# ErikBrorsson/MVDet

Hardware: AMD Instinct MI355X
Metric: multi-view frames/sec (project+fuse) (higher is better)
Workload: dtype f32 (3xbf16-split products hi*hi+hi*lo+lo*hi on the bf16 MFMA, fp32 accumulate)

## Files before the change

### mvdet_amd/csrc/conv_bf16x3.hip

```cpp
#include "common.h"

#include <type_traits>

namespace mvbev {
namespace b3 {

typedef float floatx16 __attribute__((ext_vector_type(16)));
typedef float floatx4 __attribute__((ext_vector_type(4)));
typedef __bf16 bf16x8 __attribute__((ext_vector_type(8)));
typedef unsigned int u32x4 __attribute__((ext_vector_type(4)));

constexpr int SB = MVBEV_CONV_KC;
constexpr int KC = 2 * SB;
constexpr int NKB = 9;
constexpr int BN = MVBEV_CONV_BN;
constexpr int TW = 32;
constexpr int WPART = NKB * KC * BN;
constexpr int WBYTES = 2 * WPART * 2;
constexpr int W16 = WBYTES / 16;

__global__ void pack_kernel(const float* __restrict__ w, __bf16* __restrict__ out, int Cout,
                            int Cin_w, const int32_t* __restrict__ chan_map, int K, int K_pad) {
  const int n_cot = Cout / BN;
  const int64_t total = (int64_t)(K_pad / KC) * n_cot * 2 * WPART;
// ... 1208 lines not shown
  const int col = x0 + c, r3 = 4 * ty + q;
  if (col >= W) return;
  const int base = 12 * ty + (a.dil == 1 ? 3 * q : ring_base_row<2>(q));
  int64_t roff[5];
  bool rok[5];
#pragma unroll
  for (int m = 0; m < 5; ++m) {
    const int row = a.out_row0 + base + a.dil * (m - 1), by = row - a.in_row0;
    rok[m] = row >= 0 && row < a.H && by >= 0 && by < a.in_rows;
    roff[m] = 2 * ((int64_t)by * W + col);
  }
  u32x4 raw[4][5][2];
#pragma unroll
  for (int i = 0; i < 4; ++i) {
    const int kb = kb0 + kq + 2 * i;
    const bool kok = kb < nb && g * a.group + kb * SB < a.K;
    const u32x4* src = a.x + ((int64_t)b * a.batch_stride + (int64_t)g * a.group_stride +
                              (int64_t)(kok ? kb : 0) * SB * plane) / 4;
#pragma unroll
    for (int m = 0; m < 5; ++m)
#pragma unroll
      for (int p = 0; p < 2; ++p) raw[i][m][p] = (kok && rok[m]) ? src[roff[m] + p] : u32x4{0u, 0u, 0u, 0u};
  }
#pragma unroll
  for (int i = 0; i < 4; ++i) {
    const int kb = kb0 + kq + 2 * i, k0 = g * a.group + kb * SB;
    if (kb >= nb || k0 >= a.K) continue;
    float d[5][8];
#pragma unroll
    for (int m = 0; m < 5; ++m) {
      float h[8], l[8];
      bf16x8_to_f32(raw[i][m][0], h);
      bf16x8_to_f32(raw[i][m][1], l);
#pragma unroll
      for (int j = 0; j < 8; ++j) d[m][j] = h[j] + l[j];
    }
    u32x4* dst = a.t + 2 * (((int64_t)b * K8 + k0 / SB) * R5 * W + (int64_t)5 * r3 * W) + col;
#pragma unroll
    for (int xi = 0; xi < 5; ++xi) {
      unsigned hp[4], lp[4];
#pragma unroll
      for (int e4 = 0; e4 < 4; ++e4) {
        unsigned short hs[2], ls[2];
#pragma unroll
        for (int e = 0; e < 2; ++e) {
          const int j = 2 * e4 + e;
          const float d0 = d[0][j], d1 = d[1][j], d2 = d[2][j], d3 = d[3][j], d4 = d[4][j];
          const float v = xi == 0 ? 2.f * d0 - d1 - 2.f * d2 + d3
                        : xi == 1 ? -2.f * d1 - d2 + d3
                        : xi == 2 ? 2.f * d1 - 3.f * d2 + d3
                        : xi == 3 ? d3 - d1
                                  : 2.f * d1 - d2 - 2.f * d3 + d4;
          const __bf16 hv = (__bf16)v, lv = (__bf16)(v - (float)hv);
          hs[e] = __builtin_bit_cast(unsigned short, hv);
          ls[e] = __builtin_bit_cast(unsigned short, lv);
        }
        hp[e4] = (unsigned)hs[0] | ((unsigned)hs[1] << 16);
        lp[e4] = (unsigned)ls[0] | ((unsigned)ls[1] << 16);
      }
      dst[2 * (int64_t)xi * W] = u32x4{hp[0], hp[1], hp[2], hp[3]};
      dst[2 * (int64_t)xi * W + W] = u32x4{lp[0], lp[1], lp[2], lp[3]};
    }
  }
}

#ifndef MVBEV_WINO_STAMPS
#define MVBEV_WINO_STAMPS 0
#endif
#if MVBEV_WINO_STAMPS
__device__ long long g_wino_stamps[4 * 65536];
#endif
__device__ __attribute__((always_inline)) inline void init_to_m(floatx16 (&acc)[2][wino::NXI]) {
#pragma unroll
  for (int ct = 0; ct < 2; ++ct)
#pragma unroll
    for (int r = 0; r < 16; ++r) {
      const float i0 = acc[ct][0][r], i1 = acc[ct][1][r], i2 = acc[ct][2][r];
      acc[ct][0][r] = i0 - i2;
      acc[ct][1][r] = 0.5f * (i1 + i2);
      acc[ct][2][r] = 0.5f * (i2 - i1);
    }
}

template <bool RELU, int DIL, bool P3>
__global__ __launch_bounds__(RNT, 1) void conv_wino_kernel(const Args a) {
  using namespace wino;
  using G = Geo<DIL>;
#if MVBEV_WINO_STAMPS
  const long long stamp0 = wall_clock64();
#endif
  constexpr int XW = G::XW, TROW = G::TROW, NXT = G::NXT;
  __shared__ __attribute__((aligned(16))) u32x4 lds[LDS];
  const int W = a.W;
  const int tid = threadIdx.x, lane = tid & 63;
  const int wave = __builtin_amdgcn_readfirstlane(tid >> 6);
  const int l32 = lane & 31, kl = lane >> 5;

  int tile = xcd_remap(blockIdx.x, a.nwg);
  if (a.gmask) {
    const int Gq = a.mgroup;
    const int x = blockIdx.x & 7, j = blockIdx.x >> 3;
    const int q = j / a.n_cot;
    const int slot = Gq * (8 * (q / Gq) + x) + q % Gq;
    if (slot >= a.npix) return;
    tile = (a.tile_order ? a.tile_order[slot] : slot) * a.n_cot + j % a.n_cot;
  }
  const int cot = tile % a.n_cot, rest = tile / a.n_cot;
  const int t_main = a.tiles_y * a.tiles_x;
  const int pp = rest % t_main, b = rest / t_main;
  const int ty = pp / a.tiles_x;
  const int x0 = (pp - ty * a.tiles_x) * TW;
  const int y0 = a.out_row0 + ty * RT;
  if (a.cmask && !((a.cmask[pp] >> (cot / a.cot_pg)) & 1u)) return;
  const uint32_t gm = a.gmask ? a.gmask[pp] : 0u;
  const int nch = a.gmask ? __builtin_popcount(gm) * a.cpg : a.nchunks;
  const int K8 = a.K / SB;
  const int64_t tplane2 = 2LL * (XH * a.tiles_y) * W;
  const uint32_t tplane_b = (uint32_t)(tplane2 * 16);
  constexpr uint32_t kOOB = 0x80000000u;
  uint32_t wvo[NWI], tvo[NXTMAX];
#pragma unroll
  for (int j = 0; j < NWI; ++j) {
    const int e = (j * NIW + wave) * 64 + lane;
    wvo[j] = (uint32_t)(((e / RHALF) * (NTAP * 2 * BN) + e % RHALF) * 16);
    asm volatile("" : "+v"(wvo[j]));
  }
#pragma unroll
  for (int j = 0; j < NXT; ++j) {
    const int e = (j * NIW + wave) * 64 + lane;
    const int sub = e / (TROW / 2), part = (e / (TROW / 4)) & 1, rt = (e % (TROW / 4)) / XW, c = e % XW;
    const int gx = x0 - DIL + c;
    const bool z = e >= TROW || gx < 0 || gx >= W;
    tvo[j] = z ? kOOB : (uint32_t)sub * tplane_b + (uint32_t)((2 * (XH * ty + NXI * rt) * W + part * W + gx) * 16);
    asm volatile("" : "+v"(tvo[j]));
  }
  const int cpg = a.gmask ? a.cpg : max(nch, 1);
  uint32_t rem = a.gmask ? gm : 1u;
  int gbase = a.gmask ? __builtin_ctz(gm | 0x80000000u) * cpg : 0, ci = 0, wi = 0;
  auto step = [&]() __attribute__((always_inline)) {
    if (wi + 1 < nch) {
      ++wi;
      if (++ci == cpg) {
        ci = 0;
        rem &= rem - 1;
        gbase = __builtin_ctz(rem | 0x80000000u) * cpg;
      }
    }
    return gbase + ci;
  };
  const char* wcot = reinterpret_cast<const char*>(a.wp + (int64_t)cot * wino::W16);
  const char* tb0 = reinterpret_cast<const char*>(static_cast<const u32x4*>(a.x) + (int64_t)b * K8 * tplane2);
  struct ChunkBase {
    const char* w;
    const char* t;
    bool kv1;
  };
  auto base_of = [&](int ph) __attribute__((always_inline)) {
    return ChunkBase{wcot + (int64_t)ph * a.n_cot * wino::W16 * 16, tb0 + (int64_t)(2 * ph) * tplane2 * 16,
                     2 * ph + 1 < K8};
  };
  auto issue_unit = [&](const ChunkBase& cb, int xi, int slot) __attribute__((always_inline)) {
    if (wave >= NIW) return;
    u32x4* dst = lds + slot * SLOT + wave * 64;
    const __amdgpu_buffer_rsrc_t rw =
        __builtin_amdgcn_make_buffer_rsrc(const_cast<char*>(cb.w + xi * 3 * 2 * BN * 16), (short)0, 0x7fffffff, 0x00020000);
#pragma unroll
    for (int j = 0; j < NWI; ++j)
      __builtin_amdgcn_raw_ptr_buffer_load_lds(rw, (__attribute__((address_space(3))) void*)(dst + j * NIT), 16,
                                               wvo[j], 0, 0, 0);
    const int32_t rows_b = xi * W * 32;
    const __amdgpu_buffer_rsrc_t rt = __builtin_amdgcn_make_buffer_rsrc(
        const_cast<char*>(cb.t + rows_b), (short)0, cb.kv1 ? 0x7fffffff : (int)(tplane_b - rows_b), 0x00020000);
#pragma unroll
    for (int j = 0; j < NXT; ++j)
      if ((j * NIW + wave) * 64 < TROW)
        __builtin_amdgcn_raw_ptr_buffer_load_lds(rt, (__attribute__((address_space(3))) void*)(dst + RUNIT + j * NIT),
                                                 16, tvo[j], 0, 0, 0);
  };
  ChunkBase cur = base_of(gbase + ci);
  ChunkBase nx = base_of(step());
  auto advance = [&]() __attribute__((always_inline)) {
    cur = nx;
    nx = base_of(step());
  };

  const int rg = wave & 3;
  const int cw = 64 * (wave >> 2);
  floatx16 acc[2][NXI];
#pragma unroll
  for (int i = 0; i < 2; ++i)
#pragma unroll
    for (int j = 0; j < NXI; ++j) acc[i][j] = floatx16{0};
  if constexpr (!P3) {
    if (a.init) load_init<3>(a, y0 + ring_base_row<DIL>(rg), DIL, x0 + l32, cot * BN + cw, acc);
  }
  bf16x8 fb[3][2];
  bf16x8 fa[2][2][2];
  auto fetch_b = [&](int kw, int slot) __attribute__((always_inline)) {
    const u32x4* X = lds + slot * SLOT + RUNIT + kl * (TROW / 2) + rg * XW + l32 + DIL * kw;
#pragma unroll
    for (int p = 0; p < 2; ++p) fb[kw][p] = __builtin_bit_cast(bf16x8, X[p * (TROW / 4)]);
  };
  auto fetch_a = [&](int st, int slot, int kw) __attribute__((always_inline)) {
    const u32x4* Wl = lds + slot * SLOT + kw * 2 * BN + kl * BN + cw + l32;
#pragma unroll
    for (int ct = 0; ct < 2; ++ct)
#pragma unroll
      for (int p = 0; p < 2; ++p) fa[st][ct][p] = __builtin_bit_cast(bf16x8, Wl[p * RHALF + 32 * ct]);
  };
  auto sched6 = [&](auto nreads) __attribute__((always_inline)) {
    constexpr int n = decltype(nreads)::value;
#pragma unroll
    for (int i = 0; i < 6; ++i) {
      __builtin_amdgcn_sched_group_barrier(0x008, 1, 0);
      if (i < n) __builtin_amdgcn_sched_group_barrier(0x100, (n + 5) / 6, 0);
    }
  };

  constexpr int NXT_LO = TROW / NIT;
  constexpr int WHI = (TROW % NIT + 63) / 64;
  static_assert(NXT_LO + (WHI > 0) == NXT, "T pieces");
  constexpr int NPU_HI = NWI + NXT;
  constexpr int NPU_LO = NWI + NXT_LO;
  const bool whi = wave < WHI;
#ifndef MVBEV_WINO_PB2
#define MVBEV_WINO_PB2 1
#endif
  constexpr bool PB = DIL == 2 && MVBEV_WINO_PB2;
  if (nch > 0) {
    const int U = NXI * nch;
    issue_unit(cur, 0, 0);
    issue_unit(cur, 1, 1);
    issue_unit(cur, 2, 2);
    issue_unit(cur, 3, 3);
    if (PB) {
      if (whi) asm volatile("s_waitcnt vmcnt(%0)" ::"n"(2 * NPU_HI) : "memory");
      else asm volatile("s_waitcnt vmcnt(%0)" ::"n"(2 * NPU_LO) : "memory");
    } else {
      if (whi) asm volatile("s_waitcnt vmcnt(%0)" ::"n"(3 * NPU_HI) : "memory");
      else asm volatile("s_waitcnt vmcnt(%0)" ::"n"(3 * NPU_LO) : "memory");
    }
    __builtin_amdgcn_s_barrier();
    asm volatile("" ::: "memory");
    if constexpr (!P3) init_to_m(acc);
    fetch_b(0, 0);
    fetch_b(1, 0);
    fetch_a(0, 0, 0);
#define WINO_MFMAS(AS, KW, XI)                                                                       \
  _Pragma("unroll") for (int ct = 0; ct < 2; ++ct) {                                                 \
    acc[ct][XI] = __builtin_amdgcn_mfma_f32_32x32x16_bf16(fa[AS][ct][1], fb[KW][0], acc[ct][XI], 0, 0, 0); \
    acc[ct][XI] = __builtin_amdgcn_mfma_f32_32x32x16_bf16(fa[AS][ct][0], fb[KW][1], acc[ct][XI], 0, 0, 0); \
    acc[ct][XI] = __builtin_amdgcn_mfma_f32_32x32x16_bf16(fa[AS][ct][0], fb[KW][0], acc[ct][XI], 0, 0, 0); \
  }
#define WINO_UNIT(R)                                                                                 \
  do {                                                                                               \
    constexpr int XI = (R) % 5, P = (R) & 1;                                                          \
    if (u0 + (R) >= U) break;                                                                        \
    constexpr int slot = (R) & 3, nslot = ((R) + 1) & 3;                         \
    fetch_a(P ^ 1, slot, 1);                                                                         \
    fetch_b(2, slot);                                                                                \
    WINO_MFMAS(P, 0, XI);                                                                            \
    sched6(std::integral_constant<int, 6>{});                                                        \
    fetch_a(P, slot, 2);                                                                             \
    WINO_MFMAS(P ^ 1, 1, XI);                                                                        \
    sched6(std::integral_constant<int, 4>{});                                                        \
    if (!PB) {                                                                         \
                                     \
      if (whi) asm volatile("s_waitcnt vmcnt(%0) lgkmcnt(0)" ::"n"(2 * NPU_HI) : "memory");     \
      else asm volatile("s_waitcnt vmcnt(%0) lgkmcnt(0)" ::"n"(2 * NPU_LO) : "memory");          \
      __builtin_amdgcn_s_barrier();                                                                  \
      asm volatile("" ::: "memory");                                                                 \
                      \
      issue_unit(XI == 0 ? cur : nx, (XI + 4) % 5, slot);                                            \
    } else if (P == 1) {                                                                             \
                                        \
      asm volatile("s_waitcnt vmcnt(0) lgkmcnt(0)" ::: "memory");                                   \
      __builtin_amdgcn_s_barrier();                                                                  \
      asm volatile("" ::: "memory");                                                                 \
      issue_unit(XI <= 1 ? cur : nx, (XI + 3) % 5, (u0 + (R) + 3) & 3);                              \
      issue_unit(XI == 0 ? cur : nx, (XI + 4) % 5, slot);                                            \
    }                                                                                                \
    if (XI == 4) advance();                                                                          \
    fetch_b(0, nslot);                                                                               \
    fetch_b(1, nslot);                                                                               \
    fetch_a(P ^ 1, nslot, 0);                                                                        \
    WINO_MFMAS(P, 2, XI);                                                                            \
    sched6(std::integral_constant<int, 8>{});                                                        \
  } while (0)
    for (int u0 = 0; u0 < U; u0 += 20) {
      WINO_UNIT(0); WINO_UNIT(1); WINO_UNIT(2); WINO_UNIT(3); WINO_UNIT(4);
      WINO_UNIT(5); WINO_UNIT(6); WINO_UNIT(7); WINO_UNIT(8); WINO_UNIT(9);
      WINO_UNIT(10); WINO_UNIT(11); WINO_UNIT(12); WINO_UNIT(13); WINO_UNIT(14);
      WINO_UNIT(15); WINO_UNIT(16); WINO_UNIT(17); WINO_UNIT(18); WINO_UNIT(19);
    }
#undef WINO_UNIT
#undef WINO_MFMAS
    asm volatile("s_waitcnt vmcnt(0)" ::: "memory");
  } else if constexpr (!P3) {
    init_to_m(acc);
  }
  floatx16 y[2][3];
#pragma unroll
  for (int ct = 0; ct < 2; ++ct) {
    const floatx16 m0 = acc[ct][0], m1 = acc[ct][1], m2 = acc[ct][2], m3 = acc[ct][3], m4 = acc[ct][4];
    y[ct][0] = m0 + m1 + m2 + m3;
    y[ct][1] = m1 - m2 + 2.f * m3;
    y[ct][2] = m1 + m2 + 4.f * m3 + m4;
  }
  ring_epilogue<DIL, RELU, P3, false>(a, b, y0 + ring_base_row<DIL>(rg), x0 + l32, cot, cw, y, lds);
#if MVBEV_WINO_STAMPS
  __syncthreads();
  if (threadIdx.x < 4 && blockIdx.x < 65536) {
    const long long v = threadIdx.x == 0 ? stamp0 : threadIdx.x == 1 ? wall_clock64()
                      : threadIdx.x == 2 ? (long long)__smid() : (long long)tile;
    g_wino_stamps[4 * blockIdx.x + threadIdx.x] = v;
  }
#endif
}


static int wino_rows_launch(const void* x, const mvbev_conv_desc* d, int dil, const uint32_t* group_mask, void* t,
                            size_t t_bytes, void* stream, const int32_t* gate = nullptr, int32_t gate_tag = 0) {
  if (!x || !d || !t) return MVBEV_ERR_NULL;
  if (dil != 1 && dil != 2) return MVBEV_ERR_DILATION;
  if (d->B <= 0 || d->K <= 0 || d->H <= 0 || d->W <= 0 || d->in_rows <= 0 || d->out_rows <= 0 || d->group <= 0)
    return MVBEV_ERR_RANK;
  if (d->K % SB != 0 || d->group % SB != 0 || d->K % d->group != 0) return MVBEV_ERR_SHAPE;
  if (d->out_row0 < 0 || d->out_row0 + d->out_rows > d->H || d->K / d->group > 65535 || d->B > 65535)
    return MVBEV_ERR_SHAPE;
  const int64_t tiles_y = ceil_div(d->out_rows, RT), tiles_x = ceil_div(d->W, TW);
  const int64_t need = d->B * (d->K / SB) * 5 * 4 * tiles_y * d->W * 32;
  if ((size_t)need > t_bytes || 2 * need / 32 > (int64_t)INT32_MAX * 8) return MVBEV_ERR_SHAPE;
  if (group_mask && d->K / d->group > 32) return MVBEV_ERR_SHAPE;
  if (((reinterpret_cast<uintptr_t>(x) | reinterpret_cast<uintptr_t>(t)) & 15) != 0) return MVBEV_ERR_ALIGN;
  WinoRowsArgs a;
  a.x = static_cast<const u32x4*>(x);
  a.t = static_cast<u32x4*>(t);
  a.group_stride = d->group_stride, a.batch_stride = d->batch_stride;
  a.K = (int)d->K, a.group = (int)d->group, a.H = (int)d->H, a.W = (int)d->W;
  a.in_row0 = (int)d->in_row0, a.in_rows = (int)d->in_rows, a.out_row0 = (int)d->out_row0;
  a.tiles_x = (int)tiles_x, a.tiles_y = (int)tiles_y;
  a.dil = dil;
  a.gmask = group_mask;
  a.gate = gate, a.gate_tag = gate_tag;
  const int64_t nbg = ceil_div(d->group / SB, 8);
  if ((d->K / d->group) * nbg > 65535) return MVBEV_ERR_SHAPE;
  hipLaunchKernelGGL(wino_rows_kernel, dim3((unsigned)(tiles_x * tiles_y), (unsigned)((d->K / d->group) * nbg), (unsigned)d->B),
                     dim3(256), 0, as_stream(stream), a);
  MVBEV_CHECK_LAUNCH();
  return MVBEV_OK;
}

static int wino_launch(const void* t, const mvbev_conv_desc* d, const void* w_packed, const float* bias,
                       const float* init, int64_t Cout, int relu, float* y, int y_layout,
                       const uint32_t* group_mask, const int32_t* tile_order, void* stream, int dil = 1,
                       const float* w3 = nullptr, float* p3 = nullptr, int64_t band_rows = 0,
                       const uint32_t* out_mask = nullptr, int64_t cot_pg = 1) {
  if (!t || !d || !w_packed || (!y && !p3)) return MVBEV_ERR_NULL;
  if (dil != 1 && dil != 2) return MVBEV_ERR_DILATION;
  if (p3 && (!w3 || group_mask || init)) return MVBEV_ERR_SHAPE;
  if (d->B <= 0 || d->K <= 0 || d->H <= 0 || d->W <= 0 || Cout <= 0 || d->out_rows <= 0 || d->group <= 0)
    return MVBEV_ERR_RANK;
  if (Cout % BN != 0 || d->K % SB != 0 || d->group % SB != 0 || d->K % d->group != 0) return MVBEV_ERR_SHAPE;
  if (d->out_row0 < 0 || d->out_row0 + d->out_rows > d->H || d->H > INT32_MAX / 2 || d->W > INT32_MAX / 2)
    return MVBEV_ERR_SHAPE;
  if (y_layout != MVBEV_LAYOUT_F32 && y_layout != MVBEV_LAYOUT_SPLIT_BF16 &&
      !(y_layout == MVBEV_LAYOUT_SPLIT_BF16_PIX && !p3))
    return MVBEV_ERR_SHAPE;
  if (((reinterpret_cast<uintptr_t>(w_packed) | reinterpret_cast<uintptr_t>(t)) & 15) != 0) return MVBEV_ERR_ALIGN;
  Args a{};
  a.x = t; a.wp = static_cast<const u32x4*>(w_packed); a.bias = bias; a.init = init; a.y = y;
  a.w3 = w3; a.p3 = p3;
  a.B = (int)d->B; a.group = (int)d->group; a.K = (int)d->K; a.nchunks = (int)ceil_div(d->K, KC);
  a.Cout = (int)Cout; a.H = (int)d->H; a.W = (int)d->W;
  a.in_row0 = 0; a.in_rows = (int)d->H;
  a.out_row0 = (int)d->out_row0; a.out_rows = (int)d->out_rows;
  a.tiles_x = (int)ceil_div(d->W, TW); a.tiles_y = (int)ceil_div(d->out_rows, RT);
  a.n_cot = (int)(Cout / BN);
  const int64_t tiles = (int64_t)a.tiles_x * a.tiles_y * a.n_cot * d->B;
  if (tiles > INT32_MAX / 2 || 2LL * 5 * 4 * a.tiles_y * a.W * (d->K / SB) * d->B > (int64_t)INT32_MAX * 64)
    return MVBEV_ERR_SHAPE;
  if (2LL * 32 * wino::XH * a.tiles_y * a.W >= (1LL << 31)) return MVBEV_ERR_SHAPE;
  if (group_mask) {
    if (d->group % KC != 0 || d->K / d->group > 32) return MVBEV_ERR_SHAPE;
    a.gmask = group_mask;
    a.cpg = (int)(d->group / KC);
  }
  a.tile_order = group_mask ? tile_order : nullptr;
  if (out_mask) {
    if (group_mask || p3 || band_rows || cot_pg <= 0 || a.n_cot > 32 * cot_pg) return MVBEV_ERR_SHAPE;
    a.cmask = out_mask;
    a.cot_pg = (int)cot_pg;
  }
  a.y_split = y_layout == MVBEV_LAYOUT_SPLIT_BF16 || y_layout == MVBEV_LAYOUT_SPLIT_BF16_PIX;
  a.y_pix = y_layout == MVBEV_LAYOUT_SPLIT_BF16_PIX;
  if (band_rows < 0 || (band_rows > 0 && (a.y_split || p3 || band_rows > d->out_rows))) return MVBEV_ERR_SHAPE;
  a.band_rows = (int)band_rows;
  a.npix = (int)(tiles / a.n_cot);
  a.mgroup = (group_mask && tiles >= 8 * (int64_t)std::max(cu_count(), 1)) ? 8 : 1;
  const int64_t nwg = group_mask ? (int64_t)a.n_cot * round_up(a.npix, 8 * a.mgroup) : tiles;
  a.nwg = (int)nwg;
  hipStream_t s = as_stream(stream);
  const dim3 grid((unsigned)nwg), blk(RNT);
  if (p3) {
    if (dil != 2 || !relu) return MVBEV_ERR_SHAPE;
    hipLaunchKernelGGL((conv_wino_kernel<true, 2, true>), grid, blk, 0, s, a);
  } else if (dil == 2) {
    if (relu) hipLaunchKernelGGL((conv_wino_kernel<true, 2, false>), grid, blk, 0, s, a);
    else hipLaunchKernelGGL((conv_wino_kernel<false, 2, false>), grid, blk, 0, s, a);
  } else if (relu) {
    hipLaunchKernelGGL((conv_wino_kernel<true, 1, false>), grid, blk, 0, s, a);
  } else {
    hipLaunchKernelGGL((conv_wino_kernel<false, 1, false>), grid, blk, 0, s, a);
  }
  MVBEV_CHECK_LAUNCH();
  return MVBEV_OK;
}


namespace w43 {
constexpr int NXI = 6;
constexpr int RT4 = 16;
constexpr int XH = 4 * NXI;
constexpr int NTAP = 3 * NXI;
constexpr int WPART = NTAP * KC * BN;
constexpr int W16 = 2 * WPART * 2 / 16;
template <int DIL>
__device__ inline int base_row(int rg) {
  return DIL == 1 ? 4 * rg : (rg >> 1) * 8 + (rg & 1);
}
}

__global__ void pack_wino43_kernel(const float* __restrict__ w, __bf16* __restrict__ out, int Cout, int Cin_w,
                                   const int32_t* __restrict__ chan_map, int K, int K_pad) {
  const int n_cot = Cout / BN;
  const int64_t total = (int64_t)(K_pad / KC) * n_cot * 3 * 2 * BN * SB;
  for (int64_t i = blockIdx.x * (int64_t)blockDim.x + threadIdx.x; i < total; i += (int64_t)gridDim.x * blockDim.x) {
    int64_t r = i;
    const int j = r % SB; r /= SB;
    const int co = r % BN; r /= BN;
    const int sub = r % 2; r /= 2;
    const int kw = r % 3; r /= 3;
    const int cot = r % n_cot;
    const int chunk = (int)(r / n_cot);
    const int k = chunk * KC + sub * SB + j;
    int ci = k < K ? (chan_map ? chan_map[k] : k) : -1;
    if (ci >= Cin_w) ci = -1;
    double g0 = 0.0, g1 = 0.0, g2 = 0.0;
    if (ci >= 0) {
      const float* g = w + ((int64_t)(cot * BN + co) * Cin_w + ci) * 9 + kw;
      g0 = g[0], g1 = g[3], g2 = g[6];
    }
    const double u[w43::NXI] = {0.25 * g0, -(g0 + g1 + g2) / 6.0, (g1 - g0 - g2) / 6.0,
                                g0 / 24.0 + g1 / 12.0 + g2 / 6.0, g0 / 24.0 - g1 / 12.0 + g2 / 6.0, g2};
    __bf16* o = out + ((int64_t)chunk * n_cot + cot) * 2 * w43::WPART + ((int64_t)sub * BN + co) * SB + j;
#pragma unroll
    for (int xi = 0; xi < w43::NXI; ++xi) {
      const float v = (float)u[xi];
      const __bf16 hi = (__bf16)v;
      const int tap = 3 * xi + kw;
      o[(int64_t)tap * KC * BN] = hi;
      o[(int64_t)(w43::NTAP + tap) * KC * BN] = (__bf16)(v - (float)hi);
    }
  }
}

__global__ __launch_bounds__(256) void wino43_rows_kernel(const WinoRowsArgs a) {
  constexpr int KB = 4;
  const int pp = blockIdx.x, b = blockIdx.z;
  const int nbg = (a.group / SB + KB - 1) / KB;
  const int g = blockIdx.y / nbg, kb0 = (blockIdx.y - g * nbg) * KB;
  if (a.gmask && !((a.gmask[pp] >> g) & 1u)) return;
  const int W = a.W;
  const int ty = pp / a.tiles_x;
  const int x0 = (pp - ty * a.tiles_x) * TW;
  const int nb = a.group / SB, K8 = a.K / SB, R6 = w43::NXI * 4 * a.tiles_y;
  const int64_t plane = (int64_t)a.in_rows * W;
  const int c = threadIdx.x % TW, q = (threadIdx.x / TW) % 4, kq = threadIdx.x / (4 * TW);
  const int col = x0 + c, r4 = 4 * ty + q;
  if (col >= W) return;
  const int base = w43::RT4 * ty + (a.dil == 1 ? 4 * q : (q >> 1) * 8 + (q & 1));
  int64_t roff[6];
  bool rok[6];
#pragma unroll
  for (int m = 0; m < 6; ++m) {
    const int row = a.out_row0 + base + a.dil * (m - 1), by = row - a.in_row0;
    rok[m] = row >= 0 && row < a.H && by >= 0 && by < a.in_rows;
// ... 513 lines not shown
}

size_t mvbev_conv_schedule_slot_bytes(void) { return sizeof(mvbev::b3::floatx4) * mvbev::b3::kRingSlotF4; }

int mvbev_conv3x3_dgrad_bf16x3_sched(const void* dy, int dy_layout, const mvbev_conv_desc* desc,
                                     const void* w_packed, int64_t Cout_p, int dilation, void* dx, int dx_layout,
                                     const uint32_t* out_mask, int64_t cot_per_group,
                                     const mvbev_conv_schedule* sched, void* stream) {
  using namespace mvbev::b3;
  if (!sched) return MVBEV_ERR_NULL;
  if (out_mask && (cot_per_group <= 0 || cot_per_group > 65536)) return MVBEV_ERR_SHAPE;
  if (dy_layout != MVBEV_LAYOUT_SPLIT_BF16) return MVBEV_ERR_SHAPE;
  return launch<SplitIn>(dy, desc, w_packed, nullptr, nullptr, Cout_p, dilation, 0, static_cast<float*>(dx),
                         dx_layout, nullptr, nullptr, nullptr, 0, stream, out_mask, (int)cot_per_group, nullptr,
                         nullptr, sched);
}

int mvbev_conv3x3_dgrad_bf16x3_ex(const void* dy, int dy_layout, const mvbev_conv_desc* desc, const void* w_packed,
                                  int64_t Cout_p, int dilation, void* dx, int dx_layout, const uint32_t* out_mask,
                                  int64_t cot_per_group, void* stream) {
  using namespace mvbev::b3;
  if (out_mask && (cot_per_group <= 0 || cot_per_group > 65536)) return MVBEV_ERR_SHAPE;
  if (dy_layout == MVBEV_LAYOUT_SPLIT_BF16)
    return launch<SplitIn>(dy, desc, w_packed, nullptr, nullptr, Cout_p, dilation, 0, static_cast<float*>(dx),
                           dx_layout, nullptr, nullptr, nullptr, 0, stream, out_mask, (int)cot_per_group);
  if (dy_layout != MVBEV_LAYOUT_F32) return MVBEV_ERR_SHAPE;
  return launch<float>(dy, desc, w_packed, nullptr, nullptr, Cout_p, dilation, 0, static_cast<float*>(dx),
                       dx_layout, nullptr, nullptr, nullptr, 0, stream, out_mask, (int)cot_per_group);
}

size_t mvbev_conv3x3_packed_bytes_wino(int64_t Cout, int64_t K) {
  if (Cout <= 0 || K <= 0) return 0;
  return (size_t)(mvbev::round_up(K, mvbev::b3::KC) / mvbev::b3::KC) * (size_t)(Cout / mvbev::b3::BN) *
         mvbev::b3::wino::W16 * 16;
}

int mvbev_pack_conv3x3_weight_wino_ex(const float* w, int64_t Cout, int64_t Cin_w, const int32_t* chan_map, int64_t K,
                                      void* w_packed, int32_t* nf_word, int32_t nf_tag, void* stream);

int mvbev_pack_conv3x3_weight_wino(const float* w, int64_t Cout, int64_t Cin_w, const int32_t* chan_map, int64_t K,
                                   void* w_packed, void* stream) {
  return mvbev_pack_conv3x3_weight_wino_ex(w, Cout, Cin_w, chan_map, K, w_packed, nullptr, 0, stream);
}

int mvbev_pack_conv3x3_weight_wino_ex(const float* w, int64_t Cout, int64_t Cin_w, const int32_t* chan_map, int64_t K,
                                      void* w_packed, int32_t* nf_word, int32_t nf_tag, void* stream) {
  using namespace mvbev;
  if (!w || !w_packed) return MVBEV_ERR_NULL;
  if (Cout <= 0 || Cin_w <= 0 || K <= 0) return MVBEV_ERR_RANK;
  if (Cout % b3::BN != 0) return MVBEV_ERR_SHAPE;
  if (!chan_map && K != Cin_w) return MVBEV_ERR_SHAPE;
  const int64_t total = (int64_t)mvbev_conv3x3_packed_bytes_wino(Cout, K) / 2 / (2 * b3::wino::NXI);
  const int blocks = (int)std::min<int64_t>(ceil_div(total, 256), 8192);
  hipLaunchKernelGGL(b3::pack_wino_kernel, dim3(blocks), dim3(256), 0, as_stream(stream), w,
                     static_cast<__bf16*>(w_packed), (int)Cout, (int)Cin_w, chan_map, (int)K,
                     (int)round_up(K, b3::KC), false, nf_word, nf_tag);
  MVBEV_CHECK_LAUNCH();
  return MVBEV_OK;
}

int mvbev_pack_conv3x3_weight_wino_dgrad(const float* w, int64_t Cout_f, int64_t Cin_f, int64_t Cout, void* w_packed,
                                         void* stream) {
  using namespace mvbev;
  if (!w || !w_packed) return MVBEV_ERR_NULL;
  if (Cout_f <= 0 || Cin_f <= 0 || Cout <= 0) return MVBEV_ERR_RANK;
  if (Cout % b3::BN != 0 || Cout > Cin_f || Cout_f > INT32_MAX / 2 || Cin_f > INT32_MAX / 2) return MVBEV_ERR_SHAPE;
  const int64_t total = (int64_t)mvbev_conv3x3_packed_bytes_wino(Cout, Cout_f) / 2 / (2 * b3::wino::NXI);
  const int blocks = (int)std::min<int64_t>(ceil_div(total, 256), 8192);
  hipLaunchKernelGGL(b3::pack_wino_kernel, dim3(blocks), dim3(256), 0, as_stream(stream), w,
                     static_cast<__bf16*>(w_packed), (int)Cout, (int)Cin_f, nullptr, (int)Cout_f,
                     (int)round_up(Cout_f, b3::KC), true, nullptr, 0);
  MVBEV_CHECK_LAUNCH();
  return MVBEV_OK;
}

#if MVBEV_WINO_STAMPS
int mvbev_debug_wino_stamps(void* host, size_t bytes) {
  const size_t n = std::min(bytes, sizeof(mvbev::b3::g_wino_stamps));
  return hipMemcpyFromSymbol(host, HIP_SYMBOL(mvbev::b3::g_wino_stamps), n, 0, hipMemcpyDeviceToHost) == hipSuccess
             ? MVBEV_OK : MVBEV_ERR_HIP;
}
#endif

size_t mvbev_wino_rows_bytes(const mvbev_conv_desc* d) {
  using namespace mvbev;
  if (!d || d->B <= 0 || d->K <= 0 || d->W <= 0 || d->out_rows <= 0) return 0;
  return (size_t)d->B * (size_t)(ceil_div(d->K, b3::SB)) * 5 * 4 * (size_t)ceil_div(d->out_rows, b3::RT) *
         (size_t)d->W * 32;
}

int mvbev_wino_rows_split_bf16(const void* x, const mvbev_conv_desc* desc, const uint32_t* group_mask, void* t,
                               size_t t_bytes, void* stream) {
  return mvbev::b3::wino_rows_launch(x, desc, 1, group_mask, t, t_bytes, stream);
}

int mvbev_wino_rows_split_bf16_dil(const void* x, const mvbev_conv_desc* desc, int dilation,
                                   const uint32_t* group_mask, void* t, size_t t_bytes, void* stream) {
  return mvbev::b3::wino_rows_launch(x, desc, dilation, group_mask, t, t_bytes, stream);
}

int mvbev_wino_rows_split_bf16_gated(const void* x, const mvbev_conv_desc* desc, int dilation,
                                     const uint32_t* group_mask, void* t, size_t t_bytes, const int32_t* gate,
                                     int32_t gate_tag, void* stream) {
  if (!gate) return MVBEV_ERR_NULL;
  return mvbev::b3::wino_rows_launch(x, desc, dilation, group_mask, t, t_bytes, stream, gate, gate_tag);
}

int mvbev_conv3x3_wino_bf16x3(const void* t, const mvbev_conv_desc* desc, const void* w_packed, const float* bias,
                              const float* init, int64_t Cout, int relu, void* y, int y_layout, int64_t y_band_rows,
                              const uint32_t* group_mask, const int32_t* tile_order, void* stream) {
  return mvbev::b3::wino_launch(t, desc, w_packed, bias, init, Cout, relu, static_cast<float*>(y), y_layout,
                                group_mask, tile_order, stream, 1, nullptr, nullptr, y_band_rows);
}

int mvbev_conv3x3_wino_bf16x3_dil(const void* t, const mvbev_conv_desc* desc, const void* w_packed, const float* bias,
                                  int64_t Cout, int dilation, int relu, void* y, int y_layout, void* stream) {
  return mvbev::b3::wino_launch(t, desc, w_packed, bias, nullptr, Cout, relu, static_cast<float*>(y), y_layout,
                                nullptr, nullptr, stream, dilation);
}

int mvbev_conv3x3_wino_bf16x3_dgrad(const void* t, const mvbev_conv_desc* desc, const void* w_packed, int64_t Cout,
                                    void* dx, int dx_layout, const uint32_t* out_mask, int64_t cot_per_group,
                                    void* stream) {
  if (out_mask && (cot_per_group <= 0 || cot_per_group > 65536)) return MVBEV_ERR_SHAPE;
  return mvbev::b3::wino_launch(t, desc, w_packed, nullptr, nullptr, Cout, 0, static_cast<float*>(dx), dx_layout,
                                nullptr, nullptr, stream, 1, nullptr, nullptr, 0, out_mask, cot_per_group);
}

int mvbev_conv3x3_wino_bf16x3_cout1_partials(const void* t, const mvbev_conv_desc* desc, const void* w_packed,
                                             const float* bias, int64_t Cout, int dilation, int relu, const float* w3,
                                             void* partials, size_t partials_bytes, void* stream) {
  if (!desc || !w3 || !partials) return MVBEV_ERR_NULL;
  const size_t need = mvbev_conv3x3_bf16x3_cout1_partials_bytes(desc, Cout);
  if (need == 0 || partials_bytes < need) return MVBEV_ERR_SHAPE;
  return mvbev::b3::wino_launch(t, desc, w_packed, bias, nullptr, Cout, relu, nullptr, MVBEV_LAYOUT_F32, nullptr,
                                nullptr, stream, dilation, w3, static_cast<float*>(partials));
}

}

extern "C" {

size_t mvbev_conv3x3_packed_bytes_wino43(int64_t Cout, int64_t K) {
  if (Cout <= 0 || K <= 0) return 0;
  return (size_t)(mvbev::round_up(K, mvbev::b3::KC) / mvbev::b3::KC) * (size_t)(Cout / mvbev::b3::BN) *
         mvbev::b3::w43::W16 * 16;
}

int mvbev_pack_conv3x3_weight_wino43(const float* w, int64_t Cout, int64_t Cin_w, const int32_t* chan_map, int64_t K,
                                     void* w_packed, void* stream) {
  using namespace mvbev;
  if (!w || !w_packed) return MVBEV_ERR_NULL;
  if (Cout <= 0 || Cin_w <= 0 || K <= 0) return MVBEV_ERR_RANK;
  if (Cout % b3::BN != 0) return MVBEV_ERR_SHAPE;
  if (!chan_map && K != Cin_w) return MVBEV_ERR_SHAPE;
  const int64_t total = (int64_t)mvbev_conv3x3_packed_bytes_wino43(Cout, K) / 2 / (2 * b3::w43::NXI);
  const int blocks = (int)std::min<int64_t>(ceil_div(total, 256), 8192);
  hipLaunchKernelGGL(b3::pack_wino43_kernel, dim3(blocks), dim3(256), 0, as_stream(stream), w,
                     static_cast<__bf16*>(w_packed), (int)Cout, (int)Cin_w, chan_map, (int)K,
                     (int)round_up(K, b3::KC));
  MVBEV_CHECK_LAUNCH();
  return MVBEV_OK;
}

size_t mvbev_wino43_rows_bytes(const mvbev_conv_desc* d) {
  using namespace mvbev;
// ... 29 lines not shown
```

Before: 478.6.

## Add 16x16x32 MFMA path for Winograd conv processing K-chunk pairs

Adds a variant of the Winograd conv kernel that uses the 16x16x32 bf16 MFMA instead of 32x32x16. It consumes two K chunks per step, loaded in pairs, and uses a new instruction schedule. Before the epilogue, a cross-lane bpermute fold converts the 16x16 accumulators to the existing 32x32 block layout. It is enabled by default for relu convs whose group is divisible by 2*KC, and it adds permute overhead and register pressure in exchange for possibly higher MFMA throughput and better overlap.

Measured after the change: 479.5, median of 2. Within noise of the previous version (+0.2%).

```diff
diff --git a/mvdet_amd/csrc/conv_bf16x3.hip b/mvdet_amd/csrc/conv_bf16x3.hip
--- a/mvdet_amd/csrc/conv_bf16x3.hip
+++ b/mvdet_amd/csrc/conv_bf16x3.hip
@@ -1314,10 +1314,82 @@
     }
 }
 
-template <bool RELU, int DIL, bool P3>
+__device__ __attribute__((always_inline)) inline void load_init16(const Args& a, int row_base, int dil, int col0,
+                                                                  int co0, floatx4 (&v)[4][2][wino::NXI]) {
+  const int l16 = threadIdx.x & 15, kg = (threadIdx.x & 63) >> 4;
+  const uint32_t iplane = (uint32_t)a.H * (uint32_t)a.W;
+  bool ok[3][2];
+  uint32_t roff[3][2];
+#pragma unroll
+  for (int pt = 0; pt < 3; ++pt)
+#pragma unroll
+    for (int nb = 0; nb < 2; ++nb) {
+      const int row = row_base + pt * dil, col = col0 + 16 * nb + l16;
+      ok[pt][nb] = row < a.H && col < a.W;
+      roff[pt][nb] = ok[pt][nb] ? (uint32_t)row * (uint32_t)a.W + (uint32_t)col : 0u;
+    }
+#pragma unroll
+  for (int mb = 0; mb < 4; ++mb)
+#pragma unroll
+    for (int i = 0; i < 4; ++i) {
+      const float* p = a.init + (uint32_t)(co0 + 16 * mb + 4 * kg + i) * iplane;
+#pragma unroll
+      for (int pt = 0; pt < 3; ++pt)
+#pragma unroll
+        for (int nb = 0; nb < 2; ++nb) v[mb][nb][pt][i] = ok[pt][nb] ? p[roff[pt][nb]] : 0.f;
+    }
+}
+
+__device__ __attribute__((always_inline)) inline void init_to_m16(floatx4 (&acc)[4][2][wino::NXI]) {
+#pragma unroll
+  for (int mb = 0; mb < 4; ++mb)
+#pragma unroll
+    for (int nb = 0; nb < 2; ++nb)
+#pragma unroll
+      for (int i = 0; i < 4; ++i) {
+        const float i0 = acc[mb][nb][0][i], i1 = acc[mb][nb][1][i], i2 = acc[mb][nb][2][i];
+        acc[mb][nb][0][i] = i0 - i2;
+        acc[mb][nb][1][i] = 0.5f * (i1 + i2);
+        acc[mb][nb][2][i] = 0.5f * (i2 - i1);
+      }
+}
+
+__device__ __attribute__((always_inline)) inline void fold16_to_blocks32(const floatx4 (&acc)[4][2][wino::NXI],
+                                                                         floatx16 (&y)[2][3]) {
+  const int lane = threadIdx.x & 63;
+  const int kh = lane >> 5, pb = (lane >> 4) & 1, l16 = lane & 15;
+#pragma unroll
+  for (int mb = 0; mb < 4; ++mb) {
+    floatx4 f[2][3];
+#pragma unroll
+    for (int nb = 0; nb < 2; ++nb) {
+      const floatx4 m0 = acc[mb][nb][0], m1 = acc[mb][nb][1], m2 = acc[mb][nb][2], m3 = acc[mb][nb][3],
+                    m4 = acc[mb][nb][4];
+      f[nb][0] = m0 + m1 + m2 + m3;
+      f[nb][1] = m1 - m2 + 2.f * m3;
+      f[nb][2] = m1 + m2 + 4.f * m3 + m4;
+    }
+#pragma unroll
+    for (int qb = 0; qb < 2; ++qb) {
+      const int src = 4 * (32 * qb + 16 * kh + l16);
+#pragma unroll
+      for (int pt = 0; pt < 3; ++pt)
+#pragma unroll
+        for (int e = 0; e < 4; ++e) {
+          const int v0 = __builtin_amdgcn_ds_bpermute(src, __float_as_int(f[0][pt][e]));
+          const int v1 = __builtin_amdgcn_ds_bpermute(src, __float_as_int(f[1][pt][e]));
+          y[mb >> 1][pt][4 * (2 * (mb & 1) + qb) + e] = __int_as_float(pb ? v1 : v0);
+        }
+    }
+  }
+}
+
+template <bool RELU, int DIL, bool P3, int MS = 32>
 __global__ __launch_bounds__(RNT, 1) void conv_wino_kernel(const Args a) {
   using namespace wino;
   using G = Geo<DIL>;
+  static_assert(MS == 32 || MS == 16, "MFMA shape: 32x32x16 or 16x16x32");
+  constexpr int CS = MS == 16 ? 2 : 1;
 #if MVBEV_WINO_STAMPS
   const long long stamp0 = wall_clock64();
 #endif
@@ -1370,9 +1442,9 @@
   uint32_t rem = a.gmask ? gm : 1u;
   int gbase = a.gmask ? __builtin_ctz(gm | 0x80000000u) * cpg : 0, ci = 0, wi = 0;
   auto step = [&]() __attribute__((always_inline)) {
-    if (wi + 1 < nch) {
-      ++wi;
-      if (++ci == cpg) {
+    if (wi + CS < nch) {
+      wi += CS;
+      if ((ci += CS) == cpg) {
         ci = 0;
         rem &= rem - 1;
         gbase = __builtin_ctz(rem | 0x80000000u) * cpg;
@@ -1418,43 +1490,158 @@
 
   const int rg = wave & 3;
   const int cw = 64 * (wave >> 2);
-  floatx16 acc[2][NXI];
-#pragma unroll
-  for (int i = 0; i < 2; ++i)
-#pragma unroll
-    for (int j = 0; j < NXI; ++j) acc[i][j] = floatx16{0};
-  if constexpr (!P3) {
-    if (a.init) load_init<3>(a, y0 + ring_base_row<DIL>(rg), DIL, x0 + l32, cot * BN + cw, acc);
-  }
-  bf16x8 fb[3][2];
-  bf16x8 fa[2][2][2];
-  auto fetch_b = [&](int kw, int slot) __attribute__((always_inline)) {
-    const u32x4* X = lds + slot * SLOT + RUNIT + kl * (TROW / 2) + rg * XW + l32 + DIL * kw;
-#pragma unroll
-    for (int p = 0; p < 2; ++p) fb[kw][p] = __builtin_bit_cast(bf16x8, X[p * (TROW / 4)]);
-  };
-  auto fetch_a = [&](int st, int slot, int kw) __attribute__((always_inline)) {
-    const u32x4* Wl = lds + slot * SLOT + kw * 2 * BN + kl * BN + cw + l32;
-#pragma unroll
-    for (int ct = 0; ct < 2; ++ct)
-#pragma unroll
-      for (int p = 0; p < 2; ++p) fa[st][ct][p] = __builtin_bit_cast(bf16x8, Wl[p * RHALF + 32 * ct]);
-  };
-  auto sched6 = [&](auto nreads) __attribute__((always_inline)) {
-    constexpr int n = decltype(nreads)::value;
-#pragma unroll
-    for (int i = 0; i < 6; ++i) {
-      __builtin_amdgcn_sched_group_barrier(0x008, 1, 0);
-      if (i < n) __builtin_amdgcn_sched_group_barrier(0x100, (n + 5) / 6, 0);
-    }
-  };
-
   constexpr int NXT_LO = TROW / NIT;
   constexpr int WHI = (TROW % NIT + 63) / 64;
   static_assert(NXT_LO + (WHI > 0) == NXT, "T pieces");
   constexpr int NPU_HI = NWI + NXT;
   constexpr int NPU_LO = NWI + NXT_LO;
   const bool whi = wave < WHI;
+  if constexpr (MS == 16) {
+    const int l16 = lane & 15, kg = lane >> 4;
+    floatx4 acc[4][2][NXI];
+#pragma unroll
+    for (int i = 0; i < 4; ++i)
+#pragma unroll
+      for (int j = 0; j < 2; ++j)
+#pragma unroll
+        for (int x = 0; x < NXI; ++x) acc[i][j][x] = floatx4{0.f, 0.f, 0.f, 0.f};
+    if constexpr (!P3) {
+      if (a.init) load_init16(a, y0 + ring_base_row<DIL>(rg), DIL, x0, cot * BN + cw, acc);
+    }
+    const int64_t wpair = (int64_t)a.n_cot * wino::W16 * 16, tpair = 2 * tplane2 * 16;
+    auto issue_pair = [&](const ChunkBase& cb, int xi, int dslot) __attribute__((always_inline)) {
+      issue_unit(cb, xi, dslot);
+      issue_unit(ChunkBase{cb.w + wpair, cb.t + tpair, true}, xi, dslot + 1);
+    };
+    bf16x8 fa[4][2];
+    bf16x8 fb[2][2];
+    uint32_t xo[2], wo[2];
+#pragma unroll
+    for (int d = 0; d < 2; ++d) {
+      xo[d] = (uint32_t)(((2 * d + (kg >> 1)) * SLOT + RUNIT + (kg & 1) * (TROW / 2) + rg * XW + l16) * 16);
+      wo[d] = (uint32_t)(((2 * d + (kg >> 1)) * SLOT + (kg & 1) * BN + cw + l16) * 16);
+      asm volatile("" : "+v"(xo[d]), "+v"(wo[d]));
+    }
+    const char* ldsb = reinterpret_cast<const char*>(lds);
+    auto fetch_b = [&](int nb, int dslot, int kw) __attribute__((always_inline)) {
+#pragma unroll
+      for (int p = 0; p < 2; ++p)
+        fb[nb][p] = *reinterpret_cast<const bf16x8*>(ldsb + xo[dslot >> 1] + (DIL * kw + 16 * nb + p * (TROW / 4)) * 16);
+    };
+    auto fetch_a = [&](int mb, int dslot, int kw) __attribute__((always_inline)) {
+#pragma unroll
+      for (int p = 0; p < 2; ++p)
+        fa[mb][p] = *reinterpret_cast<const bf16x8*>(ldsb + wo[dslot >> 1] + (kw * 2 * BN + 16 * mb + p * RHALF) * 16);
+    };
+    if (nch > 0) {
+      const int U = NXI * (nch / 2);
+      issue_pair(cur, 0, 0);
+      issue_pair(cur, 1, 2);
+      if (whi) asm volatile("s_waitcnt vmcnt(%0)" ::"n"(2 * NPU_HI) : "memory");
+      else asm volatile("s_waitcnt vmcnt(%0)" ::"n"(2 * NPU_LO) : "memory");
+      __builtin_amdgcn_s_barrier();
+      asm volatile("" ::: "memory");
+      if constexpr (!P3) init_to_m16(acc);
+      fetch_b(0, 0, 0);
+#pragma unroll
+      for (int mb = 0; mb < 4; ++mb) fetch_a(mb, 0, 0);
+      fetch_b(1, 0, 0);
+#define WINO16_MFMAS(M0, M1, NB, XI)                                                                               \
+  _Pragma("unroll") for (int ps = 0; ps < 3; ++ps)                                                                 \
+    _Pragma("unroll") for (int mb = M0; mb < M1; ++mb)                                                             \
+      acc[mb][NB][XI] = __builtin_amdgcn_mfma_f32_16x16x32_bf16(fa[mb][ps == 0], fb[NB][ps == 1], acc[mb][NB][XI], \
+                                                                0, 0, 0);
+#define WINO16_HEAD(XI)                                                                                             \
+  WINO16_MFMAS(0, 2, 0, XI);                                                                                       \
+  WINO16_MFMAS(0, 2, 1, XI);                                                                                       \
+  __builtin_amdgcn_sched_group_barrier(0x008, 6, 0);                                                               \
+  __builtin_amdgcn_sched_group_barrier(0x008, 6, 0)
+#define WINO16_TAIL(XI, NSLOT, NKW)                                                                                 \
+  fetch_a(0, NSLOT, NKW);                                                                                          \
+  fetch_a(1, NSLOT, NKW);                                                                                          \
+  WINO16_MFMAS(2, 4, 0, XI);                                                                                       \
+  fetch_b(0, NSLOT, NKW);                                                                                          \
+  WINO16_MFMAS(2, 4, 1, XI);                                                                                       \
+  fetch_a(2, NSLOT, NKW);                                                                                          \
+  fetch_a(3, NSLOT, NKW);                                                                                          \
+  fetch_b(1, NSLOT, NKW);                                                                                          \
+  _Pragma("unroll") for (int i = 0; i < 4; ++i) {                                                                  \
+    __builtin_amdgcn_sched_group_barrier(0x008, 1, 0);                                                             \
+    __builtin_amdgcn_sched_group_barrier(0x100, 1, 0);                                                             \
+  }                                                                                                                \
+  __builtin_amdgcn_sched_group_barrier(0x008, 2, 0);                                                               \
+  _Pragma("unroll") for (int i = 0; i < 2; ++i) {                                                                  \
+    __builtin_amdgcn_sched_group_barrier(0x008, 1, 0);                                                             \
+    __builtin_amdgcn_sched_group_barrier(0x100, 1, 0);                                                             \
+  }                                                                                                                \
+  __builtin_amdgcn_sched_group_barrier(0x008, 4, 0);                                                               \
+  __builtin_amdgcn_sched_group_barrier(0x100, 6, 0)
+#define WINO16_UNIT(R)                                                                                              \
+  do {                                                                                                             \
+    constexpr int XI = (R) % 5, dslot = 2 * ((R) & 1), nslot = 2 * (((R) + 1) & 1);                                \
+    if (u0 + (R) >= U) break;                                                                                      \
+    WINO16_HEAD(XI);                                                                                               \
+    WINO16_TAIL(XI, dslot, 1);                                                                                     \
+    WINO16_HEAD(XI);                                                                                               \
+    WINO16_TAIL(XI, dslot, 2);                                                                                     \
+    WINO16_HEAD(XI);                                                                                               \
+    __builtin_amdgcn_sched_barrier(0);           \
+            \
+    asm volatile("s_waitcnt vmcnt(0) lgkmcnt(0)" ::: "memory");                                                    \
+    __builtin_amdgcn_s_barrier();                                                                                  \
+    asm volatile("" ::: "memory");                                                                                 \
+    issue_pair(XI <= 2 ? cur : nx, (XI + 2) % 5, dslot);                                                           \
+    if (XI == 4) advance();                                                                                        \
+    WINO16_TAIL(XI, nslot, 0);                                                                                     \
+  } while (0)
+      for (int u0 = 0; u0 < U; u0 += 10) {
+        WINO16_UNIT(0); WINO16_UNIT(1); WINO16_UNIT(2); WINO16_UNIT(3); WINO16_UNIT(4);
+        WINO16_UNIT(5); WINO16_UNIT(6); WINO16_UNIT(7); WINO16_UNIT(8); WINO16_UNIT(9);
+      }
+#undef WINO16_UNIT
+#undef WINO16_TAIL
+#undef WINO16_HEAD
+#undef WINO16_MFMAS
+      asm volatile("s_waitcnt vmcnt(0)" ::: "memory");
+    } else if constexpr (!P3) {
+      init_to_m16(acc);
+    }
+    floatx16 y[2][3];
+    fold16_to_blocks32(acc, y);
+    ring_epilogue<DIL, RELU, P3, false>(a, b, y0 + ring_base_row<DIL>(rg), x0 + l32, cot, cw, y, lds);
+    return;
+  }
+  floatx16 acc[2][NXI];
+#pragma unroll
+  for (int i = 0; i < 2; ++i)
+#pragma unroll
+    for (int j = 0; j < NXI; ++j) acc[i][j] = floatx16{0};
+  if constexpr (!P3) {
+    if (a.init) load_init<3>(a, y0 + ring_base_row<DIL>(rg), DIL, x0 + l32, cot * BN + cw, acc);
+  }
+  bf16x8 fb[3][2];
+  bf16x8 fa[2][2][2];
+  auto fetch_b = [&](int kw, int slot) __attribute__((always_inline)) {
+    const u32x4* X = lds + slot * SLOT + RUNIT + kl * (TROW / 2) + rg * XW + l32 + DIL * kw;
+#pragma unroll
+    for (int p = 0; p < 2; ++p) fb[kw][p] = __builtin_bit_cast(bf16x8, X[p * (TROW / 4)]);
+  };
+  auto fetch_a = [&](int st, int slot, int kw) __attribute__((always_inline)) {
+    const u32x4* Wl = lds + slot * SLOT + kw * 2 * BN + kl * BN + cw + l32;
+#pragma unroll
+    for (int ct = 0; ct < 2; ++ct)
+#pragma unroll
+      for (int p = 0; p < 2; ++p) fa[st][ct][p] = __builtin_bit_cast(bf16x8, Wl[p * RHALF + 32 * ct]);
+  };
+  auto sched6 = [&](auto nreads) __attribute__((always_inline)) {
+    constexpr int n = decltype(nreads)::value;
+#pragma unroll
+    for (int i = 0; i < 6; ++i) {
+      __builtin_amdgcn_sched_group_barrier(0x008, 1, 0);
+      if (i < n) __builtin_amdgcn_sched_group_barrier(0x100, (n + 5) / 6, 0);
+    }
+  };
+
 #ifndef MVBEV_WINO_PB2
 #define MVBEV_WINO_PB2 1
 #endif
@@ -1583,6 +1770,12 @@
   return MVBEV_OK;
 }
 
+#ifndef MVBEV_WINO_MFMA16
+#define MVBEV_WINO_MFMA16 1
+#endif
+static int g_wino_force32 = 0;
+static int g_wino_last_shape = 0;
+
 static int wino_launch(const void* t, const mvbev_conv_desc* d, const void* w_packed, const float* bias,
                        const float* init, int64_t Cout, int relu, float* y, int y_layout,
                        const uint32_t* group_mask, const int32_t* tile_order, void* stream, int dil = 1,
@@ -1634,7 +1827,14 @@
   a.nwg = (int)nwg;
   hipStream_t s = as_stream(stream);
   const dim3 grid((unsigned)nwg), blk(RNT);
-  if (p3) {
+  const bool pairs = MVBEV_WINO_MFMA16 && !g_wino_force32 && relu && !out_mask && d->group % (2 * KC) == 0 &&
+                     (p3 ? dil == 2 : dil == 1);
+  g_wino_last_shape = pairs ? 16 : 32;
+  if (pairs && p3) {
+    hipLaunchKernelGGL((conv_wino_kernel<true, 2, true, 16>), grid, blk, 0, s, a);
+  } else if (pairs) {
+    hipLaunchKernelGGL((conv_wino_kernel<true, 1, false, 16>), grid, blk, 0, s, a);
+  } else if (p3) {
     if (dil != 2 || !relu) return MVBEV_ERR_SHAPE;
     hipLaunchKernelGGL((conv_wino_kernel<true, 2, true>), grid, blk, 0, s, a);
   } else if (dil == 2) {
@@ -2314,6 +2514,12 @@
 }
 #endif
 
+int mvbev_debug_wino_mfma_shape(void) { return mvbev::b3::g_wino_last_shape; }
+int mvbev_debug_wino_mfma_force32(int on) {
+  mvbev::b3::g_wino_force32 = on != 0;
+  return MVBEV_OK;
+}
+
 size_t mvbev_wino_rows_bytes(const mvbev_conv_desc* d) {
   using namespace mvbev;
   if (!d || d->B <= 0 || d->K <= 0 || d->W <= 0 || d->out_rows <= 0) return 0;
```
